# gabry1998/Self-Supervised-Anomaly-Detection

Hardware: AMD Instinct MI355X
Metric: train images/sec + anomaly-maps/sec, ResNet-18 256x256 bs256 (higher is better)
Workload: dtype f32; 1 GPU; ResNet-18 256x256 bs256 self-sup train + anomaly map, 1xMI355X, synthetic images (BASELINE configs[1]); images_per_gpu=256, global_batch=256, patches_per_image=841, bank_rows=588, parallelism=dp1 (256 images), train_step_launch=hipGraph segments, train_graph_segments=1

## Files before the change

### include/ssad.h

```cpp
#ifndef SSAD_H
#define SSAD_H
#include <stddef.h>
#include <stdint.h>

#ifdef __cplusplus
extern "C" {
#endif

#define SSAD_VERSION 100

int ssad_version(void);
const char* ssad_last_error(void);

int ssad_repack_oihw_to_ohwi(const float* w_oihw, float* w_ohwi, int O, int I, int KH, int KW, void* stream);
int ssad_repack_ohwi_to_oihw(const float* w_ohwi, float* w_oihw, int O, int I, int KH, int KW, void* stream);
int ssad_pack_stem_weight(const float* w_oihw, float* wk, void* stream);
int ssad_pack_stem_weight_ohwi(const float* w_ohwi, float* wk, void* stream);

int ssad_stem_fwd(const float* img, int B, int H, int W, int patch_dim, int patch_stride, int Hv, int Wv,
                  const float* wk, const float* scale, const float* shift, int relu, int hwnc, float* out, void* stream);
int ssad_stem_stats_rows(void);
int ssad_stem_fwd_stats(const float* img, int B, int H, int W, int Hv, int Wv, const float* wk, float* out, float eps,
                        float momentum, float* mean, float* invstd, float* running_mean, float* running_var, double* workspace,
                        void* stream);
// ... 34 lines not shown
int ssad_cosine_knn_mean(const float* sim, float* out, int64_t Nq, int Nb, int k, void* stream);

int ssad_blur_relu_bilinear(const float* maps, float* out, int n, int h, int w, int ksize, int target, void* stream);

int ssad_gradcam_map(const float* act, const float* alpha, float* out, int64_t B, int HW, int C, int alpha_stride,
                     void* stream);

int64_t ssad_auroc_workspace(int64_t n);
int ssad_auroc(const float* scores, const uint8_t* labels, int64_t n, void* workspace, int64_t workspace_bytes, double* out,
               void* stream);

int ssad_flip_transpose_weight(const float* w_ohwi, float* out, int O, int I, int KH, int KW, void* stream);
int ssad_flip_transpose_batch(const float* src, float* dst, const int64_t* desc, int n, void* stream);
int ssad_conv_igemm_dgrad(const float* dy, const float* w_flipT, float* dx, const float* residual, int64_t N, int Hy, int Wy,
                          int Cout, int Hx, int Wx, int Cin, int KH, int KW, int stride, int pad, void* stream);
int ssad_conv_igemm_fwd_x3(const float* in, const float* w_ohwi, float* out, const float* scale, const float* shift,
                           const float* residual, int relu, int64_t N, int H, int W, int Cin, int Cout, int KH, int KW,
                           int stride, int pad, int hwnc, void* stream);
int ssad_conv_igemm_dgrad_x3(const float* dy, const float* w_flipT, float* dx, const float* residual, int64_t N, int Hy,
                             int Wy, int Cout, int Hx, int Wx, int Cin, int KH, int KW, int stride, int pad, void* stream);
int ssad_conv_igemm_fwd_x6(const float* in, const float* w_ohwi, float* out, const float* scale, const float* shift,
                           const float* residual, int relu, int64_t N, int H, int W, int Cin, int Cout, int KH, int KW,
                           int stride, int pad, int hwnc, void* stream);
int ssad_conv_igemm_dgrad_x6(const float* dy, const float* w_flipT, float* dx, const float* residual, int64_t N, int Hy,
                             int Wy, int Cout, int Hx, int Wx, int Cin, int KH, int KW, int stride, int pad, void* stream);
int ssad_bn_small_ok(int64_t R, int C);
int ssad_bn_small_fwd(const float* z, const float* gamma, const float* beta, float* y, float* mean, float* invstd,
                      float* running_mean, float* running_var, int64_t R, int C, float eps, float momentum, int relu, void* stream);
int ssad_bn_small_bwd(const float* dy, const float* z, const float* mean, const float* invstd, const float* gamma,
                      const float* zmask_beta, float* dbeta, float* dgamma, float* dbias, float* dz, int64_t R, int C, void* stream);
// ... 349 lines not shown
```

### self-supervised-anomaly-detection_amd/csrc/conv_igemm.hip

```cpp
#include "common.h"
#include <stdlib.h>
#include <type_traits>

#ifndef IGEMM_ABL
#define IGEMM_ABL 0
#endif
#ifndef IGEMM_VAR
#define IGEMM_VAR 4
#endif
#ifndef IGEMM_EPI
#define IGEMM_EPI 1
#endif


#ifndef IGEMM_BUFLD
#define IGEMM_BUFLD 1
#endif

#ifndef IGEMM_TRACE
#define IGEMM_TRACE 0
#endif
#if IGEMM_TRACE
__device__ unsigned long long* g_ig_trace;
#define IG_STAMP(i) do { if (threadIdx.x == 0 && g_ig_trace) g_ig_trace[((size_t)blockIdx.y * gridDim.x + blockIdx.x) * 8 + (i)] = __builtin_readcyclecounter(); } while (0)
// ... 10 lines not shown
struct ConvParams {
    const float* in;
    const float* wt;
    float* out;
    const float* scale;
    const float* shift;
    const float* residual;
    const uint8_t* res_mask;
    int64_t M;
    int64_t N;
    int H, W, Cin, Ho, Wo, Cout, KH, KW, stride, pad, relu;
    int K;
    int hwnc;
    int cls_start[5];
    int cls_id[4];
    double* stats;
    int skip_lo, skip_hi;
    int pos_lpt;
    int pos_sg;
    int pos_chunk;
    unsigned char pos_tab[64];
};

template <int BM, int BN, int TM, int TN, int BK, int TS, bool POS, bool DB = true, int BF = 0, bool IO = false>
__global__ __launch_bounds__((BM / (32 * TM)) * (BN / (32 * TN)) * 64, (TM * TN > 8 || (TM * TN == 8 && BK >= 32)) ? 1 : 2)
void conv_igemm_f32_kernel(ConvParams p) {
    static_assert(!IO || BF == 2, "half tensors go with fp16 operands");
    using io_t = std::conditional_t<IO, hf, float>;
    constexpr int PE = IO ? 8 : 4;
    constexpr int NT = (BM / (32 * TM)) * (BN / (32 * TN)) * 64;
    constexpr int LDK = BF == 6 ? 3 * BK + 8 : (BF == 3 ? 2 * BK + 8 : (BF ? BK + 8 : BK + 4));
    constexpr int ESZ = BF ? 2 : 4;
    constexpr int CPR = BK / PE;
    constexpr int RPP = NT / CPR;
    constexpr int WN = BN / (32 * TN);
    constexpr int AR = BM / RPP;
    constexpr int BR = BN / RPP;
    static_assert(AR >= 1 && BR >= 1, "tile too small for the staging pattern");
    constexpr int STAGE = (BM + BN) * LDK * ESZ / 4;
    constexpr int LDC = BN + 4;
    extern __shared__ __attribute__((aligned(16))) float lds[];

    const int tid = threadIdx.x, lane = tid & 63, wave = tid >> 6;
    const int r = lane & 31, h = lane >> 5;
    const int wm = wave / WN, wn = wave % WN;
    const int n0 = blockIdx.y * BN;
    IG_STAMP(0);
#if IGEMM_TRACE
    if (threadIdx.x == 0 && g_ig_trace)
        g_ig_trace[((size_t)blockIdx.y * gridDim.x + blockIdx.x) * 8 + 7] =
            ((unsigned long long)__builtin_amdgcn_s_getreg((31 << 11) | 20) << 32) | __builtin_amdgcn_s_getreg((31 << 11) | 4);
#endif
    const int sc = tid % CPR, sr = tid / CPR;
    const int HoWo = p.Ho * p.Wo;
    const int ntaps = p.KH * p.KW;
    const int64_t in_sp = p.hwnc ? p.N * p.Cin : (int64_t)p.Cin;
    const int64_t in_sn = p.hwnc ? (int64_t)p.Cin : (int64_t)p.H * p.W * p.Cin;
    const io_t* zero = (const io_t*)g_zero_page;
    const io_t* const tin = (const io_t*)p.in;
    const io_t* const twt = (const io_t*)p.wt;

// ... 36 lines not shown
                if ((unsigned)y < (unsigned)p.H && (unsigned)x < (unsigned)p.W) tapmask |= 1u << t;
            }
    } else {
        m0 = (int64_t)blockIdx.x * BM;
    }
    int cpy = 0, cpx = 0, Hc = 1, Wc = 1;
    int64_t Mc = 0;
    if (TS > 1) {
        int c = 0;
        while (c < 3 && (int)blockIdx.x >= p.cls_start[c + 1]) ++c;
        cpy = p.cls_id[c] >> 1;
        cpx = p.cls_id[c] & 1;
        Hc = (p.Ho - cpy + 1) / 2;
        Wc = (p.Wo - cpx + 1) / 2;
        Mc = p.N * Hc * Wc;
        m0 = (int64_t)((int)blockIdx.x - p.cls_start[c]) * BM;
        tapmask = 0;
        for (int ky = 0, t = 0; ky < p.KH; ++ky)
            for (int kx = 0; kx < p.KW; ++kx, ++t)
                if (((cpy - p.pad + ky) & 1) == 0 && ((cpx - p.pad + kx) & 1) == 0) tapmask |= 1u << t;
    }
    auto decode_row = [&](int64_t m, int64_t& n, int& oy, int& ox) -> bool {
        if (TS > 1) {
            const bool ok = m < Mc;
            const int64_t mm = ok ? m : 0;
            n = mm / (Hc * Wc);
            const int rem = (int)(mm - n * (Hc * Wc));
            const int a = rem / Wc;
            oy = 2 * a + cpy;
            ox = 2 * (rem - a * Wc) + cpx;
            return ok;
// ... 65 lines not shown
                const int64_t nf = (m0 < p.M ? m0 : 0) / HoWo;
                a_org = nf * in_sn - ((int64_t)p.pad * p.W + p.pad) * in_sp;
                const int64_t R = (n - nf) * in_sn + ((int64_t)(iy0 + p.pad) * p.W + ix0 + p.pad) * in_sp + sc * PE;
                a_voff[i] = ok ? (unsigned)(R * (int64_t)sizeof(io_t)) : OOB;
            }
        }
    }
    const io_t* b_ptr[BR];
#pragma unroll
    for (int i = 0; i < BR; ++i) {
        const int co = n0 + sr + RPP * i;
        b_ptr[i] = co < p.Cout ? twt + (int64_t)co * p.K + sc * PE : nullptr;
        b_voff[i] = co < p.Cout ? (unsigned)(((int64_t)(sr + RPP * i) * p.K + sc * PE) * (int64_t)sizeof(io_t)) : OOB;
    }
    const io_t* const b_org = twt + (int64_t)n0 * p.K;

    f32x16 acc[TM][TN];
#pragma unroll
    for (int i = 0; i < TM; ++i)
#pragma unroll
        for (int j = 0; j < TN; ++j)
#pragma unroll
            for (int e = 0; e < 16; ++e) acc[i][j][e] = 0.f;

    const int cpt = p.Cin / BK;
    const int nk = __builtin_popcount(tapmask) * cpt;
    f32x4 ra2[2][AR], rb2[2][BR];
    f32x4 (&ra)[AR] = ra2[0];
    f32x4 (&rb)[BR] = rb2[0];

    unsigned ld_mask = tapmask;
    int ld_tap = tapmask ? __builtin_ctz(tapmask) : 0;
    int ld_ky = ld_tap / p.KW, ld_kx = ld_tap - ld_ky * p.KW, ld_cc = 0;
    int64_t ld_koff = 0;
    int ld_woff = 0, ld_ptap = 0, ld_pky = 0, ld_pkx = 0;
    auto load_begin = [&]() {
        if (BUFA && TS > 1)
            ld_koff = ((int64_t)((cpy - p.pad + ld_ky) >> 1) * p.W + ((cpx - p.pad + ld_kx) >> 1)) * in_sp + ld_cc * BK;
        else
            ld_koff = TS > 1 ? (int64_t)ld_cc * BK : ((int64_t)ld_ky * p.W + ld_kx) * in_sp + ld_cc * BK;
        ld_woff = (ld_tap * cpt + ld_cc) * BK;
        ld_ptap = ld_tap; ld_pky = ld_ky; ld_pkx = ld_kx;
        if (++ld_cc == cpt) {
            ld_cc = 0;
            ld_mask &= ld_mask - 1;
            if (BUFA && POS && !ld_mask) ld_mask = tapmask;
            ld_tap = ld_mask ? __builtin_ctz(ld_mask) : 0;
            ld_ky = ld_tap / p.KW;
            ld_kx = ld_tap - ld_ky * p.KW;
        }
    };
    auto load_piece = [&](int q, int set = 0) {
#if IGEMM_ABL & 64
        {
            const io_t* src;
            if (q < AR) {
                const bool ok = (a_mask[q] >> ld_ptap) & 1u;
                src = ok ? a_ptr[q] + ld_koff : zero;
            } else {
                src = b_ptr[q - AR] ? b_ptr[q - AR] + ld_woff : zero;
            }
            float* dst = lds + 2 * STAGE + ((tid >> 6) * (AR + BR) + q) * 256;
            __builtin_amdgcn_global_load_lds((const __attribute__((address_space(1))) void*)src,
                                             (__attribute__((address_space(3))) void*)dst, 16, 0, 0);
            return;
        }
#endif
        if (q < AR) {
            if constexpr (BUFA) {
                const __amdgpu_buffer_rsrc_t rs = __builtin_amdgcn_make_buffer_rsrc((void*)(tin + a_org + ld_koff), 0, (int)OOB, SRD3);
                const unsigned vo = POS ? a_voff[q] : (((a_mask[q] >> ld_ptap) & 1u) ? a_voff[q] : OOB);
                ra2[set][q] = __builtin_bit_cast(f32x4, __builtin_amdgcn_raw_buffer_load_b128(rs, vo, 0, 0));
            } else {
                const bool ok = (a_mask[q] >> ld_ptap) & 1u;
                const io_t* src = a_ptr[q] + ld_koff;
                if (TS > 1) src += ((int64_t)((a_iy[q] + ld_pky) / TS) * p.W + (a_ix[q] + ld_pkx) / TS) * in_sp;
                ra2[set][q] = *(const f32x4*)(const void*)(ok ? src : zero);
            }
        } else {
            if constexpr (BUFB) {
                const __amdgpu_buffer_rsrc_t rs = __builtin_amdgcn_make_buffer_rsrc((void*)(b_org + ld_woff), 0, (int)OOB, SRD3);
                rb2[set][q - AR] = __builtin_bit_cast(f32x4, __builtin_amdgcn_raw_buffer_load_b128(rs, b_voff[q - AR], 0, 0));
            } else {
                rb2[set][q - AR] = *(const f32x4*)(const void*)(b_ptr[q - AR] ? b_ptr[q - AR] + ld_woff : zero);
            }
        }
    };
    auto load_step = [&]() {
        load_begin();
#pragma unroll
        for (int q = 0; q < AR + BR; ++q) load_piece(q);
    };
    auto store_step = [&](float* buf) {
        if (BF == 6) {
            __bf16* As = (__bf16*)buf;
            __bf16* Bs = As + BM * LDK;
// ... 591 lines not shown
    int64_t gx = POS ? (q.pos_lpt == 2 ? cdiv64(cdiv64(q.pos_sg, 8), q.pos_chunk) * q.pos_chunk * p.Ho * p.Wo * 8
                        : q.pos_lpt ? cdiv64(q.pos_sg, q.pos_chunk) * q.pos_chunk * p.Ho * p.Wo
                                    : cdiv64(cdiv64(p.N, BM), 32) * 32 * p.Ho * p.Wo)
                     : cdiv64(p.M, BM);
    if (TS > 1) {
        int taps[4];
        for (int c = 0; c < 4; ++c) {
            taps[c] = 0;
            for (int ky = 0; ky < p.KH; ++ky)
                for (int kx = 0; kx < p.KW; ++kx)
                    taps[c] += (((c >> 1) - p.pad + ky) & 1) == 0 && (((c & 1) - p.pad + kx) & 1) == 0;
            q.cls_id[c] = c;
        }
        for (int i = 1; i < 4; ++i)
            for (int j = i; j > 0 && taps[q.cls_id[j]] > taps[q.cls_id[j - 1]]; --j) { int t = q.cls_id[j]; q.cls_id[j] = q.cls_id[j - 1]; q.cls_id[j - 1] = t; }
        gx = 0;
        for (int c = 0; c < 4; ++c) {
            q.cls_start[c] = (int)gx;
            gx += cdiv64(p.N * ((p.Ho - (q.cls_id[c] >> 1) + 1) / 2) * ((p.Wo - (q.cls_id[c] & 1) + 1) / 2), BM);
        }
        q.cls_start[4] = (int)gx;
    }
    dim3 grid((unsigned)gx, (unsigned)((p.Cout + BN - 1) / BN));
    hipLaunchKernelGGL((conv_igemm_f32_kernel<BM, BN, TM, TN, BK, TS, POS, DB, BF, IO>), grid,
                       dim3((BM / (32 * TM)) * (BN / (32 * TN)) * 64), lds_bytes, st, q);
    return (int)gx;
}

template <int TS, int BF = 1, bool IO = false>
int dispatch_bf16(const ConvParams& p, hipStream_t st) {
    if (p.Cout <= 64) return launch<256, 64, 2, 2, 32, TS, false, true, BF, IO>(p, st);
    return launch<128, 128, 2, 2, 32, TS, false, true, BF, IO>(p, st);
}

template <int TS, bool POS>
int dispatch_x6(const ConvParams& p, hipStream_t st) {
    static const int v = getenv("SSAD_X6_VARIANT") ? atoi(getenv("SSAD_X6_VARIANT")) : 1;
    if (v == 1) {
// ... 221 lines not shown
    if (posmajor_rows((IgemmEntry)mode, p)) return 100 + (int)pick_tile<true>(p);
    const IgemmTile t = pick_tile<false>(p);
    return t == T_256x256 ? T_128x128 : (int)t;
}

extern "C" int ssad_conv_igemm_tile(int64_t N, int H, int W, int Cin, int Cout, int KH, int KW, int stride, int pad, int mode) {
    static const int dims[13][3] = {{256, 64, 16}, {256, 64, 32}, {128, 64, 32}, {256, 128, 32}, {256, 128, 32}, {128, 256, 32},
                                    {64, 64, 32}, {128, 128, 32}, {256, 256, 32}, {128, 64, 32}, {128, 64, 16}, {128, 128, 16}, {128, 256, 16}};
    const int id = ssad_conv_igemm_tile_id(N, H, W, Cin, Cout, KH, KW, stride, pad, mode), t = id % 100;
    const int code = dims[t][0] * 100000 + dims[t][1] * 100 + dims[t][2];
    return id >= 100 ? -code : code;
}

static int dgrad_impl(const float* dy, const float* w_flipT, float* dx, const float* residual, int64_t N,
                                     int Hy, int Wy, int Cout, int Hx, int Wx, int Cin, int KH, int KW, int stride,
                                     int pad, void* stream, int bf16, const uint8_t* res_mask = nullptr, int io16 = 0) {
    SSAD_CHECK_ARG(dy && w_flipT && dx, "null pointer");
    SSAD_CHECK_ARG(!io16 || (bf16 == 2 && !res_mask && Cin % 4 == 0), "half tensors: fp16 operands, no residual mask, Cin % 4 == 0");
    SSAD_CHECK_ARG(N > 0 && Hy > 0 && Wy > 0 && Hx > 0 && Wx > 0 && Cin > 0 && Cout > 0, "empty shape");
    if ((bf16 == 0 || bf16 == 1 || bf16 == 2) && !io16 && !res_mask && KH == 1 && KW == 1 && Hy == 1 && Wy == 1 && Hx == 1 && Wx == 1 &&
        stride == 1 && pad == 0 && ssad_linear_small_ok(dy, w_flipT, N, Cout))
        return ssad_linear_small_launch(dy, w_flipT, dx, nullptr, nullptr, residual, 0, (int)N, Cout, Cin, nullptr, nullptr, stream, bf16);
    SSAD_CHECK_ARG(Cout % KALIGN == 0, "Cout (the contraction) must be a multiple of 32");
    SSAD_CHECK_ARG(KH > 0 && KW > 0 && pad >= 0 && pad < KH && pad < KW, "bad filter geometry");
    SSAD_CHECK_ARG(stride == 1 || stride == 2, "stride 1 or 2");
    SSAD_CHECK_ARG((Hx + 2 * pad - KH) / stride + 1 == Hy && (Wx + 2 * pad - KW) / stride + 1 == Wy, "dy/dx sizes disagree");
    SSAD_CHECK_ARG(KH == KW && KH * KW <= 32, "square filters with at most 32 taps only");
    SSAD_CHECK_ARG(!res_mask || (residual && Cin % 4 == 0), "residual mask needs a residual and Cin % 4 == 0");
    ConvParams p = dgrad_params(N, Hy, Wy, Cout, Hx, Wx, Cin, KH, KW, pad);
    p.in = dy; p.wt = w_flipT; p.out = dx; p.residual = residual; p.res_mask = res_mask;
    SSAD_CHECK_ARG(!posmajor_rows(E_DGRAD, p), "input gradients: pixel-major rows");
    SSAD_CHECK_ARG(cdiv64(p.M, 128) < (int64_t)2147483647, "M too large for one launch");
    SSAD_CHECK_ARG(tile_span_ok(p, false, io16 ? 2 : 4, stride), "gradient images too large: the rows of a tile must span less than 2 GB");
    hipStream_t st = (hipStream_t)stream;
    if (bf16 == 6) {
        if (stride == 1) dispatch_x6<1, false>(p, st);
        else dispatch_x6<2, false>(p, st);
    } else if (bf16 == 3) {
        if (stride == 1) dispatch_x3<1, false>(p, st);
        else dispatch_x3<2, false>(p, st);
    } else if (bf16 == 2 && io16) {
        if (stride == 1) dispatch_bf16<1, 2, true>(p, st);
        else dispatch_bf16<2, 2, true>(p, st);
    } else if (bf16 == 2) {
        if (stride == 1) dispatch_bf16<1, 2>(p, st);
        else dispatch_bf16<2, 2>(p, st);
    } else if (bf16) {
// ... 5 lines not shown
    return 0;
}

extern "C" int ssad_conv_igemm_dgrad(const float* dy, const float* w_flipT, float* dx, const float* residual, int64_t N,
                                     int Hy, int Wy, int Cout, int Hx, int Wx, int Cin, int KH, int KW, int stride,
                                     int pad, void* stream) {
    return dgrad_impl(dy, w_flipT, dx, residual, N, Hy, Wy, Cout, Hx, Wx, Cin, KH, KW, stride, pad, stream, 0);
}

extern "C" int ssad_conv_igemm_dgrad_masked(const float* dy, const float* w_flipT, float* dx, const float* residual,
                                            const uint8_t* res_mask, int64_t N, int Hy, int Wy, int Cout, int Hx, int Wx, int Cin,
                                            int KH, int KW, int stride, int pad, void* stream) {
    return dgrad_impl(dy, w_flipT, dx, residual, N, Hy, Wy, Cout, Hx, Wx, Cin, KH, KW, stride, pad, stream, 0, res_mask);
}

extern "C" int ssad_conv_igemm_dgrad_bf16(const float* dy, const float* w_flipT, float* dx, const float* residual, int64_t N,
                                          int Hy, int Wy, int Cout, int Hx, int Wx, int Cin, int KH, int KW, int stride,
                                          int pad, void* stream) {
    return dgrad_impl(dy, w_flipT, dx, residual, N, Hy, Wy, Cout, Hx, Wx, Cin, KH, KW, stride, pad, stream, 1);
}

extern "C" int ssad_conv_igemm_dgrad_f16(const float* dy, const float* w_flipT, float* dx, const float* residual, int64_t N,
                                         int Hy, int Wy, int Cout, int Hx, int Wx, int Cin, int KH, int KW, int stride,
                                         int pad, void* stream) {
    return dgrad_impl(dy, w_flipT, dx, residual, N, Hy, Wy, Cout, Hx, Wx, Cin, KH, KW, stride, pad, stream, 2);
}

extern "C" int ssad_conv_igemm_dgrad_x6(const float* dy, const float* w_flipT, float* dx, const float* residual, int64_t N,
                                        int Hy, int Wy, int Cout, int Hx, int Wx, int Cin, int KH, int KW, int stride,
                                        int pad, void* stream) {
// ... 33 lines not shown
```

### self-supervised-anomaly-detection_amd/self_supervised/_hip.py

```python
import ctypes
import os

import torch

_HERE = os.path.dirname(os.path.abspath(__file__))
LIB_PATH = os.path.join(os.path.dirname(_HERE), "lib", "libssad_hip.so")

_c_fp = ctypes.c_void_p
_c_i = ctypes.c_int
_c_l = ctypes.c_int64
_c_f = ctypes.c_float

SIGNATURES = {
    "ssad_repack_oihw_to_ohwi": [_c_fp, _c_fp, _c_i, _c_i, _c_i, _c_i, _c_fp],
    "ssad_repack_ohwi_to_oihw": [_c_fp, _c_fp, _c_i, _c_i, _c_i, _c_i, _c_fp],
    "ssad_pack_stem_weight": [_c_fp, _c_fp, _c_fp],
    "ssad_pack_stem_weight_ohwi": [_c_fp, _c_fp, _c_fp],
    "ssad_pack_stem_weight16_ohwi": [_c_fp, _c_fp, _c_i, _c_fp],
    "ssad_stem_fwd": [_c_fp, _c_i, _c_i, _c_i, _c_i, _c_i, _c_i, _c_i, _c_fp, _c_fp, _c_fp, _c_i, _c_i, _c_fp, _c_fp],
    "ssad_stem_stats_rows": [],
    "ssad_stem_fwd_stats": [_c_fp, _c_i, _c_i, _c_i, _c_i, _c_i, _c_fp, _c_fp, _c_f, _c_f, _c_fp, _c_fp, _c_fp, _c_fp, _c_fp, _c_fp],
    "ssad_pack_stem_weight_folded": [_c_fp, _c_fp, _c_fp],
    "ssad_stem_patch_pool_fwd": [_c_fp, _c_i, _c_i, _c_i, _c_i, _c_fp, _c_fp, _c_fp, _c_i, _c_fp, _c_fp],
    "ssad_stem_patch_pool_fwd_ring": [_c_fp, _c_i, _c_i, _c_i, _c_i, _c_fp, _c_fp, _c_fp, _c_i, _c_i, _c_i, _c_fp, _c_fp],
# ... 43 lines not shown
    "ssad_local_patch_features": [_c_fp, _c_fp, _c_fp, _c_l, _c_i, _c_i, _c_i, _c_i, _c_i, _c_i, _c_i, _c_fp],
    "ssad_stage_pyramid_rows": [_c_fp, _c_fp, _c_fp, _c_fp, _c_fp, _c_l, _c_i, _c_i, _c_i, _c_i, _c_i, _c_i, _c_i, _c_i, _c_i, _c_i, _c_i,
                                _c_i, _c_fp],
    "ssad_coreset_greedy": [_c_fp, _c_l, _c_i, _c_i, _c_l, _c_i, _c_fp, _c_fp, _c_fp, _c_fp, _c_fp, _c_fp],
    "ssad_gaussian_fit_stats": [_c_fp, _c_l, _c_i, _c_i, _c_fp, _c_fp, _c_fp, _c_fp],
    "ssad_mahalanobis_fused": [_c_fp, _c_fp, _c_fp, _c_fp, _c_fp, _c_l, _c_i, _c_i, _c_fp],
    "ssad_position_gaussian_fit_stats": [_c_fp, _c_fp, _c_i, _c_l, _c_i, _c_i, _c_fp, _c_fp, _c_fp],
    "ssad_position_mahalanobis": [_c_fp, _c_fp, _c_fp, _c_fp, _c_fp, _c_fp, _c_i, _c_l, _c_i, _c_i, _c_fp],
    "ssad_position_gaussian_factor": [_c_fp, _c_fp, _c_l, _c_i, _c_l, ctypes.c_double, _c_fp, _c_fp, _c_fp, _c_fp, _c_fp, _c_fp,
                                      _c_fp],
    "ssad_blur_relu_bilinear": [_c_fp, _c_fp, _c_i, _c_i, _c_i, _c_i, _c_i, _c_fp],
    "ssad_flip_transpose_weight": [_c_fp, _c_fp, _c_i, _c_i, _c_i, _c_i, _c_fp],
    "ssad_flip_transpose_batch": [_c_fp, _c_fp, ctypes.POINTER(ctypes.c_int64), _c_i, _c_fp],
    "ssad_conv_igemm_dgrad": [_c_fp, _c_fp, _c_fp, _c_fp, _c_l, _c_i, _c_i, _c_i, _c_i, _c_i, _c_i, _c_i, _c_i, _c_i, _c_i,
                              _c_fp],
    "ssad_bn_small_ok": [_c_l, _c_i],
    "ssad_bn_small_fwd": [_c_fp, _c_fp, _c_fp, _c_fp, _c_fp, _c_fp, _c_fp, _c_fp, _c_l, _c_i, _c_f, _c_f, _c_i, _c_fp],
    "ssad_bn_small_bwd": [_c_fp, _c_fp, _c_fp, _c_fp, _c_fp, _c_fp, _c_fp, _c_fp, _c_fp, _c_fp, _c_l, _c_i, _c_fp],
    "ssad_linear_small_max_rows": [],
    "ssad_linear_wgrad_small": [_c_fp, _c_fp, _c_fp, _c_l, _c_i, _c_i, _c_i, _c_fp],
    "ssad_linear_wgrad_small_r": [_c_fp, _c_fp, _c_fp, _c_l, _c_i, _c_i, _c_i, _c_i, _c_fp],
    "ssad_wgrad_splits": [_c_l, _c_i, _c_i, _c_i, _c_i],
    "ssad_wgrad_splits_bf16": [_c_l, _c_i, _c_i, _c_i, _c_i],
    "ssad_conv_wgrad": [_c_fp, _c_fp, _c_fp, _c_i, _c_l, _c_i, _c_i, _c_i, _c_i, _c_i, _c_i, _c_i, _c_i, _c_l, _c_fp],
    "ssad_conv_igemm_fwd_bf16": [_c_fp, _c_fp, _c_fp, _c_fp, _c_fp, _c_fp, _c_i, _c_l, _c_i, _c_i, _c_i, _c_i, _c_i, _c_i,
                                 _c_i, _c_i, _c_fp],
    "ssad_conv_igemm_fwd_x3": [_c_fp, _c_fp, _c_fp, _c_fp, _c_fp, _c_fp, _c_i, _c_l, _c_i, _c_i, _c_i, _c_i, _c_i, _c_i,
                               _c_i, _c_i, _c_i, _c_fp],
    "ssad_conv_igemm_fwd_x6": [_c_fp, _c_fp, _c_fp, _c_fp, _c_fp, _c_fp, _c_i, _c_l, _c_i, _c_i, _c_i, _c_i, _c_i, _c_i,
                               _c_i, _c_i, _c_i, _c_fp],
# ... 205 lines not shown
```

### self-supervised-anomaly-detection_amd/self_supervised/ops.py

```python
import os

import torch

from . import _hip


PROFILE = None


def _new(shape, like):
    return torch.empty(shape, device=like.device, dtype=torch.float32)


def _newh(shape, like):
    return torch.empty(shape, device=like.device, dtype=torch.float16)


def _is_h(t):
    return t is not None and t.dtype == torch.float16


def _p(t, allow_none=False):
    return _hip.ptr(t, allow_none, torch.float16 if _is_h(t) else torch.float32)

# ... 1520 lines not shown
    assert alpha.is_cuda and alpha.dtype == torch.float32
    out = _new((b, 1, u, v), act)
    _run("gradcam_map", 2.0 * act.numel(), 4.0 * act.numel(),
         lambda: _hip.lib().ssad_gradcam_map(_hip.ptr(act), alpha.data_ptr(), _hip.ptr(out), b, u * v, c, max(alpha.stride(0), c),
                                             _hip.stream()))
    return out


def flip_transpose_weight(w_ohwi):
    o, kh, kw, i = w_ohwi.shape
    out = _new((i, kh, kw, o), w_ohwi)
    _hip.check(_hip.lib().ssad_flip_transpose_weight(_hip.ptr(w_ohwi), _hip.ptr(out), o, i, kh, kw, _hip.stream()))
    return out


def conv_dgrad(dy, w_flipT, x_shape, stride, pad, residual=None, bf16=False, res_mask=None):
    n, hy, wy, cout = dy.shape
    cin, kh, kw, _ = w_flipT.shape
    assert residual is None or tuple(residual.shape) == tuple(x_shape), "residual must have dx's shape"
    assert tuple(x_shape) == (n, x_shape[1], x_shape[2], cin) and w_flipT.shape[-1] == cout
    if _is_h(dy):
        assert _is_h(w_flipT) and bf16 == 2 and res_mask is None and (residual is None or _is_h(residual))
        dx = _newh(tuple(x_shape), dy)
        _run("conv_igemm_h16", 2.0 * dx.numel() * kh * kw * cout / (stride * stride),
             2.0 * (dy.numel() + dx.numel() * (2 if residual is not None else 1) + w_flipT.numel()),
             lambda: _hip.lib().ssad_conv_igemm_dgrad_h(dy.data_ptr(), w_flipT.data_ptr(), dx.data_ptr(), _p(residual, True), n, hy, wy,
                                                        cout, x_shape[1], x_shape[2], cin, kh, kw, stride, pad, _hip.stream()))
        return dx
    dx = _new(tuple(x_shape), dy)
    if res_mask is not None:
        assert not bf16 and residual is not None
        _run("conv_igemm_f32", 2.0 * dx.numel() * kh * kw * cout / (stride * stride),
             4.0 * (dy.numel() + dx.numel() * 2 + w_flipT.numel()),
# ... 433 lines not shown
```

### self-supervised-anomaly-detection_amd/self_supervised/training.py

```python
import math
import os

import torch
import torch.distributed as dist
from torch import nn

from . import _hip, engine, ops

BN_TYPES = (nn.BatchNorm1d, nn.BatchNorm2d)


def _backward_order(model):
    out = []
    out += [model.classifier.weight, model.classifier.bias]
    ls = list(model.latent_space)
    out += [ls[-1].weight, ls[-1].bias, ls[-2].weight, ls[-2].bias]
    for seq in reversed(ls[:-2]):
        out += [seq[1].weight, seq[1].bias, seq[0].weight]
    out += [model.concatenator[1].weight, model.concatenator[1].bias, model.concatenator[0].weight]
    head_count = len(out)
    fe = model.feature_extractor
    for name, _, _, _ in reversed(engine.BLOCKS):
        for blk in reversed(list(getattr(fe, name))):
            out += [blk.bn2.weight, blk.bn2.bias, blk.conv2.weight, blk.bn1.weight, blk.bn1.bias, blk.conv1.weight]
# ... 313 lines not shown
                scale = (bn.weight * self.invstd).contiguous()
                shift = bn.bias - bn.running_mean * scale
                if bias is not None:
                    shift = shift + bias * scale
            if self._gamma_grad_under_eval_stats():
                z = ops.conv_fwd(x, w, None, a.w(bias) if bias is not None else None, None, False, self.stride, self.pad, bf)
                y = ops.bn_apply_fwd(z, self.mean, self.invstd.contiguous(), a.w(bn.weight), a.w(bn.bias), residual, self.relu)
                self.z, self.eval_stats = z, True
                self.y = y if self.relu else None
                return y
            y = ops.conv_fwd(x, w, scale, shift.contiguous(), residual, self.relu, self.stride, self.pad, bf)
            self.z = None
        self.y = y if self.relu else None
        return y

    def bwd(self, dy, need_dx=True, dx_residual=None, want_dres=False, dy_mask=None, dx_res_mask=None):
        a, bn = self.eng.arena, self.bn
        dres = None
        bias = getattr(self.lin, "bias", None)
        mask = getattr(self, "mask", None)
        if bn is None:
            dz = dy
        else:
            c = bn.num_features
            train_stats = self.z is not None and not getattr(self, "eval_stats", False)
            pg = self.eng.param_grads
            wg, bg = bn.weight.requires_grad and pg, bn.bias.requires_grad and pg
            small_bias = None
            if (train_stats and not self.is_conv and dy_mask is None and mask is None and not want_dres and not self.res_used
                    and ops.bn_small_ok(dy.numel() // c, c)):
                dbeta = a.grad(bn.bias) if bg else None
# ... 56 lines not shown
                                        res_mask=dx_res_mask)
                else:
                    assert dx_res_mask is None, "use_relu_mask16 keeps the mask away from launches csrc/conv16.hip runs"
                    dx = ops.conv3x3_h(dzz, self.eng.flipped(self.lin, wt, half=True), residual=dx_residual)
            elif (dz.dtype == torch.float32 and dz.dim() == 4 and wt is w and self.is_conv
                  and self.eng.conv32w_ok(self, dz.shape[0], dz.shape[1], dz.shape[2], cout, self.lin.in_channels)):
                dx = ops.conv3x3_hw(dzz.contiguous(), self.eng.packed_hw(self.lin, True, f32=True), self.lin.in_channels,
                                    residual=dx_residual, res_mask=dx_res_mask)
            elif self.c64_ok() and dz.dim() == 4:
                dx = ops.conv3x3_c64(dzz, self.eng.flipped(self.lin, wt), residual=dx_residual, res_mask=dx_res_mask, bf16=bf)
            elif half:
                assert dx_res_mask is None
                dx = ops.conv_dgrad(dzz, self.eng.flipped(self.lin, wt, half=True), self.x_shape, self.stride, self.pad, dx_residual, bf)
            else:
                wf = self.eng.flipped(self.lin, wt) if wt is w else ops.flip_transpose_weight(wt)
                dx = ops.conv_dgrad(dzz, wf, self.x_shape, self.stride, self.pad, dx_residual, bf, res_mask=dx_res_mask)
        self.x = self.z = self.y = self.mask = None
        return dx, dres


class _Aside:

    def __init__(self):
        self.stream, self.keep, self.dirty = None, [], False

    def launch(self, fn, keep=()):
        if self.stream is None:
            self.stream = torch.cuda.Stream()
        self.stream.wait_stream(torch.cuda.current_stream())
        with torch.cuda.stream(self.stream):
            fn()
# ... 132 lines not shown
            sizes = [e[1] * 9 * e[2] for e in entries]
            buf = torch.empty(sum(sizes), device=self.arena.p.device, dtype=torch.float32 if f32 else torch.float16)
            offs = [sum(sizes[:i]) for i in range(len(sizes))]
            tab = self._packed[key] = {"buf": buf, "entries": entries,
                                       "view": {k: buf[o:o + n] for k, o, n in zip(keys, offs, sizes)}}
        if not self._packed_ready.get(key, False):
            ops.conv3x3_hw_pack(self.arena.p, tab["entries"], out=tab["buf"], f32=f32)
            self._packed_ready[key] = True
            self._tables_used.add(("pack",) + key)
        return tab["view"][id(lin.weight)]

    def conv32w_ok(self, layer, n, h, w, cin, cout):
        l = layer.lin
        return (self.sw_conv32w and not self.bf16 and layer.is_conv and not layer.stem and l.kernel_size == (3, 3) and layer.stride == 1
                and layer.pad == 1 and l.bias is None and ops.conv3x3_hw_ok(n, h, w, cin, cout, f32=True))

    def flipped(self, lin, w, half=False):
        if half:
            return self._flipped_half(lin)
        key = id(lin.weight)
        tabs = self.__dict__.setdefault("_flip_tables", {})
        tab = tabs.get(self.h16)
        if tab is None:
            import ctypes
            a, desc, off, shapes = self.arena, [], 0, {}
            trunk = [] if self.h16 else [d[k] for d in self.blocks for k in ("c1", "c2", "ds") if d[k] is not None]
            for layer in trunk + list(self.head) + [self.cls]:
                p = layer.lin.weight
                o, c, kh, kw = p.shape if p.dim() == 4 else (p.shape[0], p.shape[1], 1, 1)
                desc += [a.offset[id(p)][0], off, o, c, kh, kw]
# ... 119 lines not shown
            if d is None:
                break
            d, _ = layer.bwd(d, need_dx=(self.trunk_grad if last else True))
        notify(a.head_end)
        if not self.trunk_grad:
            self.join_wgrad()
            self._drop_tape()
            return
        dpooled = d.view(b, -1).contiguous()
        dy = torch.empty(self.last_shape, device=dpooled.device, dtype=torch.float16 if self.h16 else torch.float32)
        ops.gap_bwd(dpooled, dy, self.gap_off["layer4"], accumulate=False)
        for i in range(len(self.blocks) - 1, -1, -1):
            blk = self.blocks[i]
            dz2_dx, dres = blk["c2"].bwd(dy, need_dx=True, want_dres=True)
            masked = isinstance(dres, tuple)
            rmask = None
            if blk["ds"] is not None:
                dx_id, _ = blk["ds"].bwd(dres[0] if masked else dres, need_dx=True, dy_mask=dres[1] if masked else None)
            elif masked:
                dx_id, rmask = dres
            else:
                dx_id = dres
            dy, _ = blk["c1"].bwd(dz2_dx, need_dx=True, dx_residual=dx_id, dx_res_mask=rmask)
            if i % 2 == 0 and i > 0:
                prev = self.blocks[i - 1]["name"]
                if prev in self.gap_off:
                    ops.gap_bwd(dpooled, dy, self.gap_off[prev], accumulate=True)
            if i % 2 == 0:
                notify(a.span[id(blk["c1"].lin.weight if blk["ds"] is None else blk["ds"].lin.weight)][1])
        self.stem.bwd_pool(self.pool_idx, dy, self.a0_shape)
        notify(a.total)
        self.join_wgrad()
        self._drop_tape()

    def head_input_grad(self, dlogits):
        b = self.batch
        pg, self.param_grads = self.param_grads, False
        try:
# ... 599 lines not shown
```

Measured before the change: 8211 images/sec.

## Fold downsample 1x1 stride-2 input gradient into the 3x3 stride-2 dgrad kernel

In ResNet downsample blocks, the 1x1 stride-2 shortcut conv's input gradient is no longer computed as its own dgrad launch and then added as a residual. It is folded into the 3x3 stride-2 implicit-GEMM dgrad as extra K-chunks, loading the second dy/weight pair only for the (0,0) parity class. The parity-class grid is also flattened into 1-D so column tiles are indexed per class. This removes a kernel launch and the write and re-read of an intermediate dx buffer. In exchange it adds branching in the load path and changes the tile scheduling of every stride-2 dgrad.

```diff
diff --git a/include/ssad.h b/include/ssad.h
--- a/include/ssad.h
+++ b/include/ssad.h
@@ -72,6 +72,9 @@
 int ssad_flip_transpose_batch(const float* src, float* dst, const int64_t* desc, int n, void* stream);
 int ssad_conv_igemm_dgrad(const float* dy, const float* w_flipT, float* dx, const float* residual, int64_t N, int Hy, int Wy,
                           int Cout, int Hx, int Wx, int Cin, int KH, int KW, int stride, int pad, void* stream);
+int ssad_conv_igemm_dgrad_fold(const float* dy, const float* w_flipT, float* dx, const float* residual, const float* dy2,
+                               const float* w2_flipT, int64_t N, int Hy, int Wy, int Cout, int Hx, int Wx, int Cin, int KH, int KW,
+                               int stride, int pad, void* stream);
 int ssad_conv_igemm_fwd_x3(const float* in, const float* w_ohwi, float* out, const float* scale, const float* shift,
                            const float* residual, int relu, int64_t N, int H, int W, int Cin, int Cout, int KH, int KW,
                            int stride, int pad, int hwnc, void* stream);
diff --git a/self-supervised-anomaly-detection_amd/csrc/conv_igemm.hip b/self-supervised-anomaly-detection_amd/csrc/conv_igemm.hip
--- a/self-supervised-anomaly-detection_amd/csrc/conv_igemm.hip
+++ b/self-supervised-anomaly-detection_amd/csrc/conv_igemm.hip
@@ -48,6 +48,9 @@
     int hwnc;
     int cls_start[5];
     int cls_id[4];
+    int cls_ny = 1;
+    const float* in2 = nullptr;
+    const float* wt2 = nullptr;
     double* stats;
     int skip_lo, skip_hi;
     int pos_lpt;
@@ -78,7 +81,7 @@
     const int tid = threadIdx.x, lane = tid & 63, wave = tid >> 6;
     const int r = lane & 31, h = lane >> 5;
     const int wm = wave / WN, wn = wave % WN;
-    const int n0 = blockIdx.y * BN;
+    int n0 = blockIdx.y * BN;
     IG_STAMP(0);
 #if IGEMM_TRACE
     if (threadIdx.x == 0 && g_ig_trace)
@@ -145,7 +148,9 @@
         Hc = (p.Ho - cpy + 1) / 2;
         Wc = (p.Wo - cpx + 1) / 2;
         Mc = p.N * Hc * Wc;
-        m0 = (int64_t)((int)blockIdx.x - p.cls_start[c]) * BM;
+        const int local = (int)blockIdx.x - p.cls_start[c], rt = __builtin_amdgcn_readfirstlane(local / p.cls_ny);
+        m0 = (int64_t)rt * BM;
+        n0 = (local - rt * p.cls_ny) * BN;
         tapmask = 0;
         for (int ky = 0, t = 0; ky < p.KH; ++ky)
             for (int kx = 0; kx < p.KW; ++kx, ++t)
@@ -241,6 +246,8 @@
         b_voff[i] = co < p.Cout ? (unsigned)(((int64_t)(sr + RPP * i) * p.K + sc * PE) * (int64_t)sizeof(io_t)) : OOB;
     }
     const io_t* const b_org = twt + (int64_t)n0 * p.K;
+    const io_t* const tin2 = (const io_t*)p.in2;
+    const io_t* const b_org2 = (const io_t*)p.wt2 + (int64_t)n0 * p.Cin;
 
     f32x16 acc[TM][TN];
 #pragma unroll
@@ -251,7 +258,11 @@
             for (int e = 0; e < 16; ++e) acc[i][j][e] = 0.f;
 
     const int cpt = p.Cin / BK;
-    const int nk = __builtin_popcount(tapmask) * cpt;
+    const bool fold = TS > 1 && p.in2 && cpy == 0 && cpx == 0;
+    const int nk1 = __builtin_popcount(tapmask) * cpt;
+    const int nk = nk1 + (fold ? cpt : 0);
+    int ld_left = fold ? nk1 : -1;
+    int ld_tcpt = cpt;
     f32x4 ra2[2][AR], rb2[2][BR];
     f32x4 (&ra)[AR] = ra2[0];
     f32x4 (&rb)[BR] = rb2[0];
@@ -262,11 +273,27 @@
     int64_t ld_koff = 0;
     int ld_woff = 0, ld_ptap = 0, ld_pky = 0, ld_pkx = 0;
     auto load_begin = [&]() {
+        if constexpr (TS > 1) {
+            if (ld_left == 0) {
+                ld_tcpt = 0;
+                ld_mask = tapmask;
+                ld_tap = __builtin_ctz(tapmask);
+                ld_ky = ld_tap / p.KW;
+                ld_kx = ld_tap - ld_ky * p.KW;
+#pragma unroll
+                for (int i = 0; i < BR; ++i) {
+                    const bool row = n0 + sr + RPP * i < p.Cout;
+                    b_ptr[i] = row ? b_org2 + (int64_t)(sr + RPP * i) * p.Cin + sc * PE : nullptr;
+                    b_voff[i] = row ? (unsigned)(((int64_t)(sr + RPP * i) * p.Cin + sc * PE) * (int64_t)sizeof(io_t)) : OOB;
+                }
+            }
+            --ld_left;
+        }
         if (BUFA && TS > 1)
             ld_koff = ((int64_t)((cpy - p.pad + ld_ky) >> 1) * p.W + ((cpx - p.pad + ld_kx) >> 1)) * in_sp + ld_cc * BK;
         else
             ld_koff = TS > 1 ? (int64_t)ld_cc * BK : ((int64_t)ld_ky * p.W + ld_kx) * in_sp + ld_cc * BK;
-        ld_woff = (ld_tap * cpt + ld_cc) * BK;
+        ld_woff = (ld_tap * (TS > 1 ? ld_tcpt : cpt) + ld_cc) * BK;
         ld_ptap = ld_tap; ld_pky = ld_ky; ld_pkx = ld_kx;
         if (++ld_cc == cpt) {
             ld_cc = 0;
@@ -295,18 +322,18 @@
 #endif
         if (q < AR) {
             if constexpr (BUFA) {
-                const __amdgpu_buffer_rsrc_t rs = __builtin_amdgcn_make_buffer_rsrc((void*)(tin + a_org + ld_koff), 0, (int)OOB, SRD3);
+                const __amdgpu_buffer_rsrc_t rs = __builtin_amdgcn_make_buffer_rsrc((void*)(((TS > 1 && !ld_tcpt) ? tin2 : tin) + a_org + ld_koff), 0, (int)OOB, SRD3);
                 const unsigned vo = POS ? a_voff[q] : (((a_mask[q] >> ld_ptap) & 1u) ? a_voff[q] : OOB);
                 ra2[set][q] = __builtin_bit_cast(f32x4, __builtin_amdgcn_raw_buffer_load_b128(rs, vo, 0, 0));
             } else {
                 const bool ok = (a_mask[q] >> ld_ptap) & 1u;
-                const io_t* src = a_ptr[q] + ld_koff;
+                const io_t* src = a_ptr[q] + ((TS > 1 && !ld_tcpt) ? tin2 - tin : 0) + ld_koff;
                 if (TS > 1) src += ((int64_t)((a_iy[q] + ld_pky) / TS) * p.W + (a_ix[q] + ld_pkx) / TS) * in_sp;
                 ra2[set][q] = *(const f32x4*)(const void*)(ok ? src : zero);
             }
         } else {
             if constexpr (BUFB) {
-                const __amdgpu_buffer_rsrc_t rs = __builtin_amdgcn_make_buffer_rsrc((void*)(b_org + ld_woff), 0, (int)OOB, SRD3);
+                const __amdgpu_buffer_rsrc_t rs = __builtin_amdgcn_make_buffer_rsrc((void*)(((TS > 1 && !ld_tcpt) ? b_org2 : b_org) + ld_woff), 0, (int)OOB, SRD3);
                 rb2[set][q - AR] = __builtin_bit_cast(f32x4, __builtin_amdgcn_raw_buffer_load_b128(rs, b_voff[q - AR], 0, 0));
             } else {
                 rb2[set][q - AR] = *(const f32x4*)(const void*)(b_ptr[q - AR] ? b_ptr[q - AR] + ld_woff : zero);
@@ -928,14 +955,15 @@
         }
         for (int i = 1; i < 4; ++i)
             for (int j = i; j > 0 && taps[q.cls_id[j]] > taps[q.cls_id[j - 1]]; --j) { int t = q.cls_id[j]; q.cls_id[j] = q.cls_id[j - 1]; q.cls_id[j - 1] = t; }
+        q.cls_ny = (p.Cout + BN - 1) / BN;
         gx = 0;
         for (int c = 0; c < 4; ++c) {
-            q.cls_start[c] = (int)gx;
+            q.cls_start[c] = (int)gx * q.cls_ny;
             gx += cdiv64(p.N * ((p.Ho - (q.cls_id[c] >> 1) + 1) / 2) * ((p.Wo - (q.cls_id[c] & 1) + 1) / 2), BM);
         }
-        q.cls_start[4] = (int)gx;
-    }
-    dim3 grid((unsigned)gx, (unsigned)((p.Cout + BN - 1) / BN));
+        q.cls_start[4] = (int)gx * q.cls_ny;
+    }
+    dim3 grid(TS > 1 ? (unsigned)(gx * q.cls_ny) : (unsigned)gx, TS > 1 ? 1u : (unsigned)((p.Cout + BN - 1) / BN));
     hipLaunchKernelGGL((conv_igemm_f32_kernel<BM, BN, TM, TN, BK, TS, POS, DB, BF, IO>), grid,
                        dim3((BM / (32 * TM)) * (BN / (32 * TN)) * 64), lds_bytes, st, q);
     return (int)gx;
@@ -1187,8 +1215,12 @@
 
 static int dgrad_impl(const float* dy, const float* w_flipT, float* dx, const float* residual, int64_t N,
                                      int Hy, int Wy, int Cout, int Hx, int Wx, int Cin, int KH, int KW, int stride,
-                                     int pad, void* stream, int bf16, const uint8_t* res_mask = nullptr, int io16 = 0) {
+                                     int pad, void* stream, int bf16, const uint8_t* res_mask = nullptr, int io16 = 0,
+                                     const float* dy2 = nullptr, const float* w2_flipT = nullptr) {
     SSAD_CHECK_ARG(dy && w_flipT && dx, "null pointer");
+    SSAD_CHECK_ARG(!dy2 == !w2_flipT, "the folded operands come as a pair");
+    SSAD_CHECK_ARG(!dy2 || (bf16 == 0 && !io16 && stride == 2 && KH == 3 && KW == 3 && pad == 1),
+                   "a folded 1 x 1 / stride 2 gradient: exact fp32, beside a 3 x 3 / stride 2 / pad 1 conv only");
     SSAD_CHECK_ARG(!io16 || (bf16 == 2 && !res_mask && Cin % 4 == 0), "half tensors: fp16 operands, no residual mask, Cin % 4 == 0");
     SSAD_CHECK_ARG(N > 0 && Hy > 0 && Wy > 0 && Hx > 0 && Wx > 0 && Cin > 0 && Cout > 0, "empty shape");
     if ((bf16 == 0 || bf16 == 1 || bf16 == 2) && !io16 && !res_mask && KH == 1 && KW == 1 && Hy == 1 && Wy == 1 && Hx == 1 && Wx == 1 &&
@@ -1202,8 +1234,10 @@
     SSAD_CHECK_ARG(!res_mask || (residual && Cin % 4 == 0), "residual mask needs a residual and Cin % 4 == 0");
     ConvParams p = dgrad_params(N, Hy, Wy, Cout, Hx, Wx, Cin, KH, KW, pad);
     p.in = dy; p.wt = w_flipT; p.out = dx; p.residual = residual; p.res_mask = res_mask;
+    p.in2 = dy2; p.wt2 = w2_flipT;
     SSAD_CHECK_ARG(!posmajor_rows(E_DGRAD, p), "input gradients: pixel-major rows");
     SSAD_CHECK_ARG(cdiv64(p.M, 128) < (int64_t)2147483647, "M too large for one launch");
+    SSAD_CHECK_ARG(stride == 1 || (cdiv64(p.M, 64) + 4) * cdiv64(Cin, 64) < (int64_t)2147483647, "too many tiles for one launch");
     SSAD_CHECK_ARG(tile_span_ok(p, false, io16 ? 2 : 4, stride), "gradient images too large: the rows of a tile must span less than 2 GB");
     hipStream_t st = (hipStream_t)stream;
     if (bf16 == 6) {
@@ -1239,6 +1273,12 @@
     return dgrad_impl(dy, w_flipT, dx, residual, N, Hy, Wy, Cout, Hx, Wx, Cin, KH, KW, stride, pad, stream, 0, res_mask);
 }
 
+extern "C" int ssad_conv_igemm_dgrad_fold(const float* dy, const float* w_flipT, float* dx, const float* residual, const float* dy2,
+                                          const float* w2_flipT, int64_t N, int Hy, int Wy, int Cout, int Hx, int Wx, int Cin, int KH,
+                                          int KW, int stride, int pad, void* stream) {
+    return dgrad_impl(dy, w_flipT, dx, residual, N, Hy, Wy, Cout, Hx, Wx, Cin, KH, KW, stride, pad, stream, 0, nullptr, 0, dy2, w2_flipT);
+}
+
 extern "C" int ssad_conv_igemm_dgrad_bf16(const float* dy, const float* w_flipT, float* dx, const float* residual, int64_t N,
                                           int Hy, int Wy, int Cout, int Hx, int Wx, int Cin, int KH, int KW, int stride,
                                           int pad, void* stream) {
diff --git a/self-supervised-anomaly-detection_amd/self_supervised/_hip.py b/self-supervised-anomaly-detection_amd/self_supervised/_hip.py
--- a/self-supervised-anomaly-detection_amd/self_supervised/_hip.py
+++ b/self-supervised-anomaly-detection_amd/self_supervised/_hip.py
@@ -81,6 +81,8 @@
     "ssad_flip_transpose_batch": [_c_fp, _c_fp, ctypes.POINTER(ctypes.c_int64), _c_i, _c_fp],
     "ssad_conv_igemm_dgrad": [_c_fp, _c_fp, _c_fp, _c_fp, _c_l, _c_i, _c_i, _c_i, _c_i, _c_i, _c_i, _c_i, _c_i, _c_i, _c_i,
                               _c_fp],
+    "ssad_conv_igemm_dgrad_fold": [_c_fp, _c_fp, _c_fp, _c_fp, _c_fp, _c_fp, _c_l, _c_i, _c_i, _c_i, _c_i, _c_i, _c_i, _c_i, _c_i,
+                                   _c_i, _c_i, _c_fp],
     "ssad_bn_small_ok": [_c_l, _c_i],
     "ssad_bn_small_fwd": [_c_fp, _c_fp, _c_fp, _c_fp, _c_fp, _c_fp, _c_fp, _c_fp, _c_l, _c_i, _c_f, _c_f, _c_i, _c_fp],
     "ssad_bn_small_bwd": [_c_fp, _c_fp, _c_fp, _c_fp, _c_fp, _c_fp, _c_fp, _c_fp, _c_fp, _c_fp, _c_l, _c_i, _c_fp],
diff --git a/self-supervised-anomaly-detection_amd/self_supervised/ops.py b/self-supervised-anomaly-detection_amd/self_supervised/ops.py
--- a/self-supervised-anomaly-detection_amd/self_supervised/ops.py
+++ b/self-supervised-anomaly-detection_amd/self_supervised/ops.py
@@ -1558,9 +1558,28 @@
     return out
 
 
-def conv_dgrad(dy, w_flipT, x_shape, stride, pad, residual=None, bf16=False, res_mask=None):
+def s2_fold_on():
+    return os.environ.get("SSAD_S2_FOLD", "1") != "0"
+
+
+def conv_dgrad(dy, w_flipT, x_shape, stride, pad, residual=None, bf16=False, res_mask=None, fold=None):
     n, hy, wy, cout = dy.shape
     cin, kh, kw, _ = w_flipT.shape
+    if fold is not None:
+        dy2, w2 = fold
+        assert not bf16 and res_mask is None and not _is_h(dy) and (stride, pad, kh, kw) == (2, 1, 3, 3)
+        assert tuple(dy2.shape) == tuple(dy.shape) and tuple(w2.shape) == (cin, 1, 1, cout)
+        if not s2_fold_on():
+            assert residual is None
+            return conv_dgrad(dy, w_flipT, x_shape, stride, pad, conv_dgrad(dy2, w2, x_shape, 2, 0))
+        dx = _new(tuple(x_shape), dy)
+        _run("conv_igemm_f32", 2.0 * dx.numel() * (kh * kw + 1) * cout / (stride * stride),
+             4.0 * (dy.numel() + dy2.numel() + dx.numel() * (2 if residual is not None else 1) + w_flipT.numel() + w2.numel()),
+             lambda: _hip.lib().ssad_conv_igemm_dgrad_fold(_hip.ptr(dy), _hip.ptr(w_flipT), _hip.ptr(dx), _hip.ptr(residual, True),
+                                                           _hip.ptr(dy2), _hip.ptr(w2), n, hy, wy, cout, x_shape[1], x_shape[2], cin,
+                                                           kh, kw, stride, pad, _hip.stream()),
+             tile=lambda: igemm_tile_name(n, x_shape[1], x_shape[2], cin, cout, kh, kw, stride, pad, IGEMM_DGRAD))
+        return dx
     assert residual is None or tuple(residual.shape) == tuple(x_shape), "residual must have dx's shape"
     assert tuple(x_shape) == (n, x_shape[1], x_shape[2], cin) and w_flipT.shape[-1] == cout
     if _is_h(dy):
diff --git a/self-supervised-anomaly-detection_amd/self_supervised/training.py b/self-supervised-anomaly-detection_amd/self_supervised/training.py
--- a/self-supervised-anomaly-detection_amd/self_supervised/training.py
+++ b/self-supervised-anomaly-detection_amd/self_supervised/training.py
@@ -351,7 +351,7 @@
         self.y = y if self.relu else None
         return y
 
-    def bwd(self, dy, need_dx=True, dx_residual=None, want_dres=False, dy_mask=None, dx_res_mask=None):
+    def bwd(self, dy, need_dx=True, dx_residual=None, want_dres=False, dy_mask=None, dx_res_mask=None, dx_fold=None, want_dz=False):
         a, bn = self.eng.arena, self.bn
         dres = None
         bias = getattr(self.lin, "bias", None)
@@ -438,7 +438,11 @@
                 dx = ops.conv_dgrad(dzz, self.eng.flipped(self.lin, wt, half=True), self.x_shape, self.stride, self.pad, dx_residual, bf)
             else:
                 wf = self.eng.flipped(self.lin, wt) if wt is w else ops.flip_transpose_weight(wt)
-                dx = ops.conv_dgrad(dzz, wf, self.x_shape, self.stride, self.pad, dx_residual, bf, res_mask=dx_res_mask)
+                dx = ops.conv_dgrad(dzz, wf, self.x_shape, self.stride, self.pad, dx_residual, bf, res_mask=dx_res_mask, fold=dx_fold)
+                dx_fold = None
+        assert dx_fold is None, "dx_fold: the implicit-GEMM input gradient only (TrainEngine.s2_fold_ok)"
+        if want_dz and not need_dx:
+            dx = dz
         self.x = self.z = self.y = self.mask = None
         return dx, dres
 
@@ -601,6 +605,12 @@
         l = layer.lin
         return (self.sw_conv32w and not self.bf16 and layer.is_conv and not layer.stem and l.kernel_size == (3, 3) and layer.stride == 1
                 and layer.pad == 1 and l.bias is None and ops.conv3x3_hw_ok(n, h, w, cin, cout, f32=True))
+
+    def s2_fold_ok(self, blk):
+        c1, ds = blk["c1"], blk["ds"]
+        return (not self.bf16 and not self.h16 and c1.is_conv and ds.is_conv and c1.lin.kernel_size == (3, 3) and c1.stride == 2
+                and c1.pad == 1 and ds.lin.kernel_size == (1, 1) and ds.stride == 2 and ds.pad == 0
+                and ds.lin.out_channels == c1.lin.out_channels and c1.lin.out_channels % 32 == 0)
 
     def flipped(self, lin, w, half=False):
         if half:
@@ -750,14 +760,17 @@
             blk = self.blocks[i]
             dz2_dx, dres = blk["c2"].bwd(dy, need_dx=True, want_dres=True)
             masked = isinstance(dres, tuple)
-            rmask = None
-            if blk["ds"] is not None:
+            rmask = fold = None
+            if blk["ds"] is not None and self.s2_fold_ok(blk):
+                dz_ds, _ = blk["ds"].bwd(dres[0] if masked else dres, need_dx=False, dy_mask=dres[1] if masked else None, want_dz=True)
+                fold, dx_id = (dz_ds, self.flipped(blk["ds"].lin, blk["ds"].weight())), None
+            elif blk["ds"] is not None:
                 dx_id, _ = blk["ds"].bwd(dres[0] if masked else dres, need_dx=True, dy_mask=dres[1] if masked else None)
             elif masked:
                 dx_id, rmask = dres
             else:
                 dx_id = dres
-            dy, _ = blk["c1"].bwd(dz2_dx, need_dx=True, dx_residual=dx_id, dx_res_mask=rmask)
+            dy, _ = blk["c1"].bwd(dz2_dx, need_dx=True, dx_residual=dx_id, dx_res_mask=rmask, dx_fold=fold)
             if i % 2 == 0 and i > 0:
                 prev = self.blocks[i - 1]["name"]
                 if prev in self.gap_off:
```

After: 8257 images/sec (median of 6 runs). About the same (+0.6%).
